# thegenemyers/DEXTRACTOR

Measured on NVIDIA B200. Metric: dexqv+undexqv uncompressed GB/s, higher is better.
Workload: dtype u8

## Files before the change

### dextractor_b200/csrc/dx_api.cpp

```cpp

#include <stdarg.h>
#include <stdio.h>
#include <stdlib.h>
#include <string.h>
#include <vector>
#include <algorithm>
#include <chrono>
#include "dx_internal.h"
#include "dx_chain.h"

struct DxPhases
{ bool on; std::chrono::steady_clock::time_point t0; char buf[512]; size_t len;
  explicit DxPhases(const dx_ctx *ctx) : on(ctx->route[DXR_DEBUG] != 0), len(0) { buf[0] = 0; t0 = std::chrono::steady_clock::now(); }
  void mark(const char *what)
  { if (!on) return;
    auto t1 = std::chrono::steady_clock::now();
    len += (size_t) snprintf(buf+len,sizeof(buf)-len," %s %.3f",what,
                             std::chrono::duration<double,std::milli>(t1-t0).count());
    if (len >= sizeof(buf)) len = sizeof(buf)-1;
    t0 = t1;
  }
  void report(const char *call) { if (on) fprintf(stderr,"[dexb200 debug] %s host phases (ms):%s\n",call,buf); }
};

// ... 114 lines not shown
void dx_prof_begin(dx_ctx *ctx)
{ DxProf *pv = (DxProf *) ctx->prof;
  DxProfRec r; r.name = NULL;
  r.a = pv->get(); r.b = pv->get();
  cudaEventRecord(r.a,ctx->stream);
  pv->push_back(r);
}

void dx_prof_end(dx_ctx *ctx, const char *what)
{ DxProf *pv = (DxProf *) ctx->prof;
  if (pv->empty() || pv->back().name != NULL) return;
  pv->back().name = what;
  cudaEventRecord(pv->back().b,ctx->stream);
}

extern "C" int dx_profile(dx_ctx *ctx, int enable)
{ if (ctx == NULL) return DX_E_ARG;
  if (ctx->prof == NULL) ctx->prof = new DxProf();
  ctx->prof_on = enable ? 1 : 0;
  return DX_OK;
}

extern "C" int dx_profile_report(dx_ctx *ctx, char *buf, size_t cap)
{ if (ctx == NULL || buf == NULL || cap == 0) return DX_E_ARG;
  buf[0] = '\0';
  if (ctx->prof == NULL) return DX_OK;
  DX_CUDA(ctx,cudaStreamSynchronize(ctx->stream));
  DxProf *pv = (DxProf *) ctx->prof;
  struct Acc { const char *name; int calls; double ms; };
  std::vector<Acc> acc;
  for (DxProfRec &r : *pv)
    { float ms = 0;
      if (r.name != NULL && cudaEventElapsedTime(&ms,r.a,r.b) == cudaSuccess)
        { size_t k = 0;
          while (k < acc.size() && strcmp(acc[k].name,r.name) != 0) k++;
          if (k == acc.size()) acc.push_back(Acc{r.name,0,0.0});
          acc[k].calls += 1; acc[k].ms += ms;
        }
      pv->pool.push_back(r.a); pv->pool.push_back(r.b);
    }
  pv->clear();
  size_t at = 0;
  for (const Acc &a : acc)
    { int w = snprintf(buf+at,cap-at,"%s %d %.6f\n",a.name,a.calls,a.ms);
      if (w < 0 || (size_t) w >= cap-at) return dx_fail(ctx,DX_E_CAP,"profile report needs more than %zu bytes",cap);
      at += (size_t) w;
    }
  return DX_OK;
}

extern "C" int dx_open(int device, dx_ctx **out)
{ if (out == NULL) return DX_E_ARG;
  *out = NULL;
  int ndev = 0;
  if (cudaGetDeviceCount(&ndev) != cudaSuccess || ndev <= 0)
    { cudaGetLastError();
      return DX_E_NOGPU;
    }
  if (device < 0 || device >= ndev) return DX_E_ARG;
  if (cudaSetDevice(device) != cudaSuccess) return DX_E_CUDA;
  dx_ctx *ctx = (dx_ctx *) calloc(1,sizeof(dx_ctx));
  if (ctx == NULL) return DX_E_NOMEM;
  ctx->device = device;
  cudaDeviceProp prop;
  if (cudaGetDeviceProperties(&prop,device) != cudaSuccess ||
      cudaStreamCreateWithFlags(&ctx->stream,cudaStreamNonBlocking) != cudaSuccess)
    { free(ctx);
      return DX_E_CUDA;
    }
  ctx->sm_count = prop.multiProcessorCount;
  ctx->route[DXR_DEBUG] = (getenv("DEXB200_DEBUG") != NULL);
  *out = ctx;
  return DX_OK;
}

extern "C" void dx_close(dx_ctx *ctx)
{ if (ctx == NULL) return;
  cudaSetDevice(ctx->device);
  cudaStreamSynchronize(ctx->stream);
  for (int i = 0; i < ctx->nblk; i++) cudaFree(ctx->blk[i].p);
  if (ctx->io_in)    cudaFree(ctx->io_in);
  if (ctx->io_out)   cudaFree(ctx->io_out);
  if (ctx->qv_store) cudaFree(ctx->qv_store);
  if (ctx->last_index) delete (std::vector<dx_index_row> *) ctx->last_index;
  if (ctx->hpin)     cudaFreeHost(ctx->hpin);
  while (ctx->hpin_extra)
    { DxPinExtra *e = (DxPinExtra *) ctx->hpin_extra; ctx->hpin_extra = e->next; cudaFreeHost(e->p); free(e); }
  if (ctx->prof)
    { char tmp[16]; ctx->prof_on = 0; dx_profile_report(ctx,tmp,sizeof(tmp));
      for (cudaEvent_t e : ((DxProf *) ctx->prof)->pool) cudaEventDestroy(e);
      delete (DxProf *) ctx->prof;
    }
  for (int i = 0; i < ctx->npev; i++) cudaEventDestroy(ctx->pev[i]);
  if (ctx->cs_in)  cudaStreamDestroy(ctx->cs_in);
  if (ctx->cs_out) cudaStreamDestroy(ctx->cs_out);
  cudaStreamDestroy(ctx->stream);
  free(ctx);
}

extern "C" const char *dx_strerror(const dx_ctx *ctx) { return ctx ? ctx->err : "no context"; }
extern "C" int64_t     dx_error_line(const dx_ctx *ctx) { return ctx ? ctx->err_line : 0; }
extern "C" size_t      dx_needed_bytes(const dx_ctx *ctx) { return ctx ? ctx->need_bytes : 0; }
extern "C" void       *dx_stream(dx_ctx *ctx) { return ctx ? (void *) ctx->stream : NULL; }

extern "C" int dx_route(dx_ctx *ctx, const char *name, int64_t value)
{ static const char *names[DXR_COUNT] = { "no_fast", "no_spec", "exact_index", "exact_pack", "pack2", "two_pass",
                                          "chain_scan", "decoder", "lane_max_rlen", "lane_min_entries", "debug",
                                          "serial_io", "pipe_chunk", "no_direct", "index_bulk", "hist_mode" };
  if (ctx == NULL || name == NULL) return DX_E_ARG;
  if (strcmp(name,"default") == 0)
    { const int64_t dbg = ctx->route[DXR_DEBUG];
      memset(ctx->route,0,sizeof(ctx->route));
      ctx->route[DXR_DEBUG] = dbg;
      return DX_OK;
    }
  for (int k = 0; k < DXR_COUNT; k++)
    if (strcmp(name,names[k]) == 0) { ctx->route[k] = value; return DX_OK; }
  return dx_fail(ctx,DX_E_ARG,"dx_route: unknown route '%s'",name);
}

extern "C" int dx_keep_index(dx_ctx *ctx, int keep)
{ if (ctx == NULL) return DX_E_ARG;
  ctx->keep_index = keep;
  if (ctx->last_index == NULL) ctx->last_index = new std::vector<dx_index_row>();
  return DX_OK;
}

extern "C" int dx_last_index(dx_ctx *ctx, dx_index_row *rows, int64_t max, int64_t *count)
{ if (ctx == NULL || count == NULL) return DX_E_ARG;
  std::vector<dx_index_row> *v = (std::vector<dx_index_row> *) ctx->last_index;
  *count = v ? (int64_t) v->size() : 0;
  if (v && rows)
    for (int64_t i = 0; i < *count && i < max; i++) rows[i] = (*v)[(size_t) i];
  return DX_OK;
}

extern "C" int dx_sync(dx_ctx *ctx)
{ DX_CUDA(ctx,cudaStreamSynchronize(ctx->stream));
  return DX_OK;
}

extern "C" uint64_t dx_launch_count(dx_ctx *ctx, int reset)
{ uint64_t v = ctx->launches;
  if (reset) ctx->launches = 0;
  return v;
}

extern "C" void *dx_device_alloc(dx_ctx *ctx, size_t bytes)
{ void *p = NULL;
  cudaSetDevice(ctx->device);
  cudaError_t e = cudaMalloc(&p,round_up(bytes + 64,256));
  if (e != cudaSuccess) { dx_cuda_fail(ctx,e,"cudaMalloc"); return NULL; }
  return p;
}
extern "C" void dx_device_free(dx_ctx *ctx, void *p) { (void) ctx; if (p) cudaFree(p); }

extern "C" void *dx_pinned_alloc(dx_ctx *ctx, size_t bytes)
{ void *p = NULL;
  cudaError_t e = cudaHostAlloc(&p,bytes > 0 ? bytes : 1,cudaHostAllocDefault);
  if (e != cudaSuccess) { dx_cuda_fail(ctx,e,"cudaHostAlloc"); return NULL; }
  return p;
}
extern "C" void dx_pinned_free(dx_ctx *ctx, void *p) { (void) ctx; if (p) cudaFreeHost(p); }

extern "C" int dx_h2d(dx_ctx *ctx, void *d, const void *h, size_t n)
{ DX_CUDA(ctx,cudaMemcpyAsync(d,h,n,cudaMemcpyHostToDevice,ctx->stream)); return DX_OK; }
extern "C" int dx_d2d(dx_ctx *ctx, void *d_dst, const void *d_src, size_t n)
{ if (ctx == NULL) return DX_E_ARG;
  cudaSetDevice(ctx->device);
  if (n > 0) DX_CUDA(ctx,cudaMemcpyAsync(d_dst,d_src,n,cudaMemcpyDeviceToDevice,ctx->stream));
  return DX_OK;
}
extern "C" int dx_d2h(dx_ctx *ctx, void *h, const void *d, size_t n)
{ DX_CUDA(ctx,cudaMemcpyAsync(h,d,n,cudaMemcpyDeviceToHost,ctx->stream)); return DX_OK; }


static int check_buf(dx_ctx *ctx, const void *p, const char *what)
{ if (p == NULL) return dx_fail(ctx,DX_E_ARG,"%s is NULL",what);
  if (((uintptr_t) p & 15) != 0)
    return dx_fail(ctx,DX_E_ARG,"%s must be 16-byte aligned device memory",what);
  return DX_OK;
}

static int peek(dx_ctx *ctx, const uint8_t *d, size_t n, size_t at, size_t len, std::vector<uint8_t> &h)
{ if (at > n) at = n;
  if (at + len > n) len = n - at;
  h.resize(len);
  if (len == 0) return DX_OK;
  DX_CUDA(ctx,cudaMemcpyAsync(h.data(),d+at,len,cudaMemcpyDeviceToHost,ctx->stream));
  DX_CUDA(ctx,cudaStreamSynchronize(ctx->stream));
  return DX_OK;
// ... 2059 lines not shown
```

### dextractor_b200/csrc/dx_internal.h

```cpp
#ifndef DX_INTERNAL_H
#define DX_INTERNAL_H

#include <stdint.h>
#include <stddef.h>
#include <cuda_runtime.h>
#include "dexb200.h"


struct QvEntries
{ int64_t  n;
  int64_t *hdr;
  int64_t *line0;
  int32_t *rlen;
  int32_t *well, *beg, *end, *qv;
  int32_t *flag;
  int32_t *order;
};

struct QvSizes
{ uint32_t *bytes;
  int64_t  *off;
};

#define DX_ENC_CODE(e)  ((e) & 0xffffu)
#define DX_ENC_LEN(e)   (((e) >> 16) & 0x1fu)
#define DX_ENC_ESC(e)   (((e) >> 21) & 1u)

struct QvEncTables { uint32_t t[6][256]; };

struct QvDecTables
{ uint8_t look[6][65536];
  uint8_t lens[6][256];
  int32_t type[6];
};

#define DX_DEC2_MAXSUB 64
struct QvDecTables2
{ uint16_t prim[6][2048];
  uint16_t sub[6][DX_DEC2_MAXSUB*32];
  int32_t  type[6];
};

struct QvDecTables4
{ uint32_t multi[6][4096];
  uint16_t single[6][4096];
  float    abits[6];
  QvDecTables2 t2;
  uint32_t longs[6][256];
  int32_t  nlong[6];
};


struct DxBlock { uint8_t *p; size_t cap, top; };

enum { DXR_NO_FAST = 0, DXR_NO_SPEC, DXR_EXACT_INDEX, DXR_EXACT_PACK, DXR_PACK2, DXR_TWO_PASS, DXR_CHAIN_SCAN,
       DXR_DECODER,
       DXR_LANE_MAX_RLEN,
       DXR_LANE_MIN_ENTRIES,
       DXR_DEBUG, DXR_SERIAL_IO,
       DXR_PIPE_CHUNK,
       DXR_NO_DIRECT,
       DXR_INDEX_BULK,
       DXR_HIST_MODE,
       DXR_COUNT };

struct dx_ctx
{ int          device;
  cudaStream_t stream;
  int          sm_count;
  char         err[512];
  int64_t      err_line;
  uint64_t     launches;
  int64_t      route[DXR_COUNT];

  DxBlock      blk[32];
  int          nblk;

  uint8_t     *io_in;   size_t io_in_cap;
  uint8_t     *io_out;  size_t io_out_cap;
  size_t       need_bytes;
  cudaStream_t cs_in, cs_out;
  void       (*overlap_fn)(void *);
  void        *overlap_arg;
  cudaEvent_t  pev[40];
  int          npev;

  int          prof_on;
  void        *prof;

  uint8_t     *hpin;    size_t hpin_cap, hpin_top, hpin_want;
  void        *hpin_extra;

  int          keep_index;
  void        *last_index;

  const uint8_t *qv_text;
  size_t         qv_n;
  QvEntries      qv_ent;
  uint8_t       *qv_store;
  size_t         qv_store_cap;
};

int   dx_fail(dx_ctx *ctx, int code, const char *fmt, ...);
int   dx_cuda_fail(dx_ctx *ctx, cudaError_t e, const char *what);
int   dx_fail_cap(dx_ctx *ctx, size_t need, size_t cap);
void  dx_arena_reset(dx_ctx *ctx);
void *dx_arena_get(dx_ctx *ctx, size_t bytes);
int   dx_arena_reserve(dx_ctx *ctx, size_t bytes);
void *dx_hpin_get(dx_ctx *ctx, size_t bytes);

#define DX_CUDA(ctx, call) do { cudaError_t e__ = (call); \
    if (e__ != cudaSuccess) return dx_cuda_fail(ctx, e__, #call); } while (0)
void dx_prof_begin(dx_ctx *ctx);
void dx_prof_end(dx_ctx *ctx, const char *what);
#define DX_PROF_BEGIN(ctx) do { if ((ctx)->prof_on) dx_prof_begin(ctx); } while (0)
#define DX_LAUNCHED(ctx, what) do { (ctx)->launches++; cudaError_t e__ = cudaGetLastError(); \
    if ((ctx)->prof_on) dx_prof_end(ctx, what); \
    if (e__ != cudaSuccess) return dx_cuda_fail(ctx, e__, what); } while (0)


int dxk_fetch(dx_ctx *ctx, void *h_pinned, const void *d_src, size_t bytes);

enum { DX_PRED_NEWLINE = 0, DX_PRED_FASTA_HDR = 1, DX_PRED_QVCAND = 2, DX_PRED_ARCAND = 3 };
int dxk_index_positions(dx_ctx *ctx, int pred, const uint8_t *d_buf, size_t n, size_t first,
                        int64_t **d_pos, int64_t *count);
int dxk_ticket_order(dx_ctx *ctx, const int32_t *d_rlen, int64_t n, int32_t *d_order);
int dxk_qv_entries(dx_ctx *ctx, const uint8_t *d_text, size_t n, const int64_t *d_nl,
                   int64_t nlines, QvEntries ent, int32_t *h_err, uint64_t *h_totchar,
                   int64_t *h_noncanon, int64_t *h_last_nl);

struct QvProbe
{ int32_t  delchar, subchar;
  int64_t  e_del, e_sub;
  uint64_t sub_prefix[256];
  uint64_t totchar;
};
int dxk_qv_probe(dx_ctx *ctx, const uint8_t *d_text, QvEntries ent, const dx_qv_carry *carry,
                 QvProbe *h_probe);
int dxk_qv_hist(dx_ctx *ctx, const uint8_t *d_text, QvEntries ent, const QvProbe *h_probe,
                uint64_t *h_hist , int32_t *h_newline_inside);

int dxk_qv_encode(dx_ctx *ctx, const uint8_t *d_text, size_t text_n, QvEntries ent,
                  const QvEncTables *h_tab,
                  int delchar, int subchar, int lossy, int32_t lwell_in,
                  uint8_t *d_out, size_t cap, size_t *out_len, int32_t *last_well,
                  int64_t *h_entry_off, int64_t max_entries);

struct QvDecEntry
{ int64_t out_off;
  int64_t text_off;
  int32_t well, beg, end, qv;
};
int dxk_qv_walk(dx_ctx *ctx, const uint8_t *d_in, size_t n, const QvDecTables *d_tab,
                int delchar, int subchar, int flip, const int64_t *d_start, const int32_t *d_rlen,
                int64_t count, int64_t *d_soff, int32_t *d_status );
int dxk_qv_decode(dx_ctx *ctx, const uint8_t *d_in, size_t n, const QvDecTables *d_tab,
                  int delchar, int subchar, int flip, int upper, const QvDecEntry *d_ent,
                  const int64_t *d_soff, int64_t count, const char *d_prefix, int plen,
                  uint8_t *d_out, int32_t *d_status );

int dxk_qv_decode5(dx_ctx *ctx, const uint8_t *d_in, size_t n, const QvDecTables4 *d_tab,
                   int delchar, int subchar, int upper, int write, int64_t count,
                   const int64_t *d_start, const int32_t *d_rlen, const QvDecEntry *d_ent,
                   const char *d_prefix, int plen, uint8_t *d_out, int64_t *d_soff, int32_t *d_status);

int dxk_qv_decode5x(dx_ctx *ctx, const uint8_t *d_in, size_t n, const QvDecTables4 *d_tab,
                    int delchar, int subchar, int upper, int write, int64_t count,
                    const int64_t *d_start, const int32_t *d_rlen, const QvDecEntry *d_ent,
                    const char *d_prefix, int plen, uint8_t *d_out, int64_t *d_soff, int32_t *d_status,
                    const int64_t *d_limit, const int32_t *d_order, const int64_t *d_toff,
                    const int64_t *d_endat = NULL);

int dxk_qv_decode6x(dx_ctx *ctx, const uint8_t *d_in, size_t n, const QvDecTables4 *d_tab,
                    int delchar, int subchar, int upper, int write, int64_t count,
                    const int64_t *d_start, const int32_t *d_rlen, const QvDecEntry *d_ent,
                    const char *d_prefix, int plen, uint8_t *d_out, int64_t *d_soff, int32_t *d_status,
                    const int64_t *d_limit, const int32_t *d_order, const int64_t *d_toff, int64_t n_coop,
                    const int64_t *d_endat = NULL);

int dxk_qv_assemble(dx_ctx *ctx, const uint8_t *d_tmp, size_t tmp_n, const QvDecEntry *d_ent,
                    const int64_t *d_src, int64_t count, const char *d_prefix, int plen, uint8_t *d_out);

struct QvPlanArrays
// ... 92 lines not shown
```

### dextractor_b200/csrc/dx_qv_decode5.cu

```cuda

#include <stdio.h>
#include <stdlib.h>
#include "dx_internal.h"
#include "dx_common.cuh"

namespace {

constexpr int kWarps    = 32;
constexpr int kThreads  = kWarps * 32;
constexpr int kS        = 256;
constexpr int kSW       = kS / 32;
constexpr int kRegion   = kSW + 1;
constexpr int kStage    = 2560;
constexpr int kTail     = 24;
constexpr int kFingerBudget = 24;

struct Dec5Args
{ const uint8_t *in;
  int64_t        n;
  const QvDecTables4 *tab;
  int32_t        delchar, subchar, upper, write;
  int64_t        count;
  const int64_t *start;
  const int32_t *rlen;
  const QvDecEntry *ent;
  const int64_t *toff;
  const char    *prefix; int32_t plen;
  uint8_t       *out;
  int64_t       *soff;
  int32_t       *status;
  const int64_t *limit;
  const int32_t *order;
  const int64_t *endat;
  unsigned long long *ticket;
  unsigned long long *dbg;
};

struct WarpMem
{ uint64_t bits[32*kRegion];
  uint32_t stage[kStage/4 + 4];
};

struct Shared5
{ uint32_t tab[4][4096];
  WarpMem  w[kWarps];
};

extern __shared__ __align__(16) uint8_t dx_dec5_smem[];

__device__ __forceinline__ uint32_t win32(const uint64_t *D, uint32_t pos)
{ const uint64_t v = D[pos >> 5];
  return __funnelshift_l((uint32_t) v,(uint32_t) (v >> 32),pos);
}

__device__ __forceinline__ uint32_t lookup_long(const QvDecTables2 *t, int k, uint32_t w16)
{ uint32_t e = __ldg(&t->prim[k][w16 >> 5]);
  if (e & 0x8000u)
    e = __ldg(&t->sub[k][(e & 0x7fffu)*32u + (w16 & 31u)]);
  return e;
}

__device__ __noinline__ uint32_t long_entry(const QvDecTables2 *t, int k, uint32_t w, uint32_t *bad)
{ const uint32_t f = lookup_long(t,k,w >> 16);
  uint32_t len = (f >> 8) & 31u;
  const uint32_t c = f & 0xffu;
  if (len == 0) { len = 1; *bad = 1; }
  if (t->type[k] == 2 && c == 255u)
    return (len + 8u) | (1u << 5) | 0x80u | (len << 8) | (255u << 16);
  return len | (1u << 5) | (len << 8) | (c << 16);
}

__device__ __noinline__ uint32_t long_single(const QvDecTables2 *t, int k, uint32_t w, uint32_t *bad)
{ uint32_t f = lookup_long(t,k,w >> 16) & 0x1fffu;
  if ((f >> 8) == 0u) { f |= 0x100u; *bad = 1; }
  return f;
}

__device__ __forceinline__ void fill_line(uint8_t *dst, uint32_t c, uint32_t n, uint32_t lane)
{ uint32_t head = (16u - (uint32_t) (reinterpret_cast<uintptr_t>(dst) & 15u)) & 15u;
  if (head > n) head = n;
  if (lane < head) dst[lane] = (uint8_t) c;
  const uint32_t nvec = (n - head) >> 4;
  const uint32_t q = c * 0x01010101u;
  const uint4 v = make_uint4(q,q,q,q);
  uint8_t *body = dst + head;
  for (uint32_t i = lane; i < nvec; i += 32) dx_stg16(body + (size_t) i*16,v);
  const uint32_t done = head + nvec*16u;
  if (lane < n - done) dst[done + lane] = (uint8_t) c;
}

__device__ __forceinline__ void stage_window(const Dec5Args &a, uint64_t *bits, const uint8_t *p,
                                             uint32_t lane, uint32_t nact)
{ if (lane < nact)
    { const uintptr_t A = reinterpret_cast<uintptr_t>(p) + 32u*lane;
      const uint32_t *al = reinterpret_cast<const uint32_t *>(A & ~(uintptr_t) 3);
      const uint32_t sh = (uint32_t) (A & 3) * 8;
      const uint32_t *endw = reinterpret_cast<const uint32_t *>(
                               (reinterpret_cast<uintptr_t>(a.in + a.n) + 3) & ~(uintptr_t) 3);
      uint32_t x[kRegion + 2];
#pragma unroll
      for (int k = 0; k < kRegion + 2; k++) x[k] = (al + k < endw) ? __ldg(al + k) : 0u;
#pragma unroll
      for (int k = 0; k < kRegion; k++)
        { const uint32_t w0 = __funnelshift_r(x[k],x[k+1],sh), w1 = __funnelshift_r(x[k+1],x[k+2],sh);
          bits[kRegion*lane + k] = ((uint64_t) w0 << 32) | w1;
        }
    }
  __syncwarp();
}

#define DX_E_LEN(e)   ((e) & 31u)
#define DX_E_N(e)     (((e) >> 5) & 3u)
#define DX_E_LEN0(e)  (((e) >> 8) & 31u)
#define DX_E_LEN1(e)  (((e) & 0x40u) ? DX_E_LEN0(e) : DX_E_LEN(e))

struct StreamOut { uint32_t bytes, kept, bad; };

template <bool RUN>
__device__ __noinline__ StreamOut decode_stream(const Dec5Args &a, int slot, int64_t so, int32_t rlen,
                                                int symtab, int runtab, int32_t rci, uint8_t *dst,
                                                int64_t budget)
{ Shared5 &sm = *reinterpret_cast<Shared5 *>(dx_dec5_smem);
  const uint32_t lane = threadIdx.x & 31u, warp = threadIdx.x >> 5;
  StreamOut res; res.bytes = 0; res.kept = 0; res.bad = 0;
  if (rlen <= 0)
    { if (dst != NULL && lane == 0) dst[0] = '\n';
      return res;
    }
  const QvDecTables2 *t2 = &a.tab->t2;
  const bool esc = (t2->type[symtab] == 2);
  const uint32_t rc = (uint32_t) rci;
  const uint32_t base = lane * kS, lim = base + kS;
  const float abits = a.tab->abits[symtab] * 1.2f;
  WarpMem &wm = sm.w[warp];
  const uint64_t *D = wm.bits + lane;
  const uint32_t *mt = sm.tab[slot];
  const uint16_t *rt = reinterpret_cast<const uint16_t *>(sm.tab[slot]), *st = rt + 4096;
  uint32_t done = 0;
  uint32_t carry = 0;
  uint32_t wword = 0;
  uint32_t bd = 0, sp = 0, ksum = 0;
  bool redecode = false;
  if (RUN && dst != NULL) fill_line(dst,rc,(uint32_t) rlen,lane);

  while (true)
    { const uint32_t remaining = (uint32_t) rlen - done;
      uint32_t nact = (uint32_t) ((float) remaining * abits * (1.0f/kS)) + 2u;
      if (nact > 32u) nact = 32u;
      const bool active = (lane < nact);
      __syncwarp();
      stage_window(a,wm.bits,a.in + so + (int64_t) wword*4,lane,nact);

      uint32_t mystart = (lane == 0) ? carry : (base << 1);
      uint32_t myexit = 0, n = 0, nk = 0;
      if (active)
        { uint32_t pos = mystart >> 1, cnt = 0, kept = 0;
          if (RUN)
            { uint32_t par = mystart & 1u;
              while (pos < lim)
                { if (par == 0)
                    { uint32_t w = win32(D,pos);
                      uint32_t e = rt[w >> 20];
                      if (e == 0u) e = long_single(t2,runtab,w,&sp);
                      uint32_t r = e & 0xffu;
                      pos += e >> 8;
                      if (r == 255u) { r = win32(D,pos) >> 16; pos += 16; }
                      cnt += r;
                      par = 1;
                      if (pos >= lim) break;
                    }
                  uint32_t w = win32(D,pos);
                  uint32_t e = st[w >> 20];
                  if (e == 0u) e = long_single(t2,symtab,w,&sp);
                  uint32_t c = e & 0xffu;
                  pos += e >> 8;
                  if (esc && c == 255u) { c = win32(D,pos) >> 24; pos += 8; }
                  cnt += 1;
                  kept += (c != rc);
                  par = 0;
                }
              myexit = (pos << 1) | par;
            }
          else
            { const uint32_t limf = lim - kTail;
              while (pos < limf)
                { const uint32_t w = win32(D,pos);
                  uint32_t e = mt[w >> 20];
                  if (e == 0u) e = long_entry(t2,symtab,w,&sp);
                  pos += DX_E_LEN(e);
                  cnt += DX_E_N(e);
                }
              while (pos < lim)
                { const uint32_t w = win32(D,pos);
                  uint32_t e = mt[w >> 20];
                  if (e == 0u) e = long_entry(t2,symtab,w,&sp);
                  pos += DX_E_LEN1(e);
                  cnt += 1;
                }
              myexit = pos << 1;
            }
          n = cnt; nk = kept;
        }

      uint32_t rounds = 0, restarts = 0, slow = 0;
      bool giveup = false;
      while (true)
        { int changed = 0;
          uint32_t want = __shfl_up_sync(DX_FULL,myexit,1);
          if (!active || lane == 0) want = mystart;
          if (want != mystart)
            { uint32_t pa = mystart >> 1, pb = want >> 1, ca = 0, cb = 0, ka = 0, kb = 0;
              restarts++;
              if (RUN)
                { uint32_t qa = mystart & 1u, qb = want & 1u;
                  while (!(pa == pb && qa == qb) && min(pa,pb) < lim)
                    { const bool fa = (pa <= pb);
                      uint32_t pos = fa ? pa : pb, par = fa ? qa : qb, dc, dk = 0;
                      if (par == 0)
                        { uint32_t w = win32(D,pos);
                          uint32_t e = rt[w >> 20];
                          if (e == 0u) e = long_single(t2,runtab,w,&sp);
                          dc = e & 0xffu;
                          pos += e >> 8;
                          if (dc == 255u) { dc = win32(D,pos) >> 16; pos += 16; }
                          par = 1;
                        }
                      else
                        { uint32_t w = win32(D,pos);
                          uint32_t e = st[w >> 20];
                          if (e == 0u) e = long_single(t2,symtab,w,&sp);
                          uint32_t c = e & 0xffu;
                          pos += e >> 8;
                          if (esc && c == 255u) { c = win32(D,pos) >> 24; pos += 8; }
                          dc = 1; dk = (c != rc);
                          par = 0;
                        }
                      if (fa) { pa = pos; qa = par; ca += dc; ka += dk; }
                      else    { pb = pos; qb = par; cb += dc; kb += dk; }
                    }
                  if (pa == pb && qa == qb) { n += cb - ca; nk += kb - ka; }
                  else { n = cb; nk = kb; myexit = (pb << 1) | qb; changed = 1; }
                }
              else if (redecode)
                {
                  uint32_t pos = want >> 1, cnt = 0;
                  const uint32_t limf = lim - kTail;
                  while (pos < limf)
                    { const uint32_t w = win32(D,pos);
                      uint32_t e = mt[w >> 20];
                      if (e == 0u) e = long_entry(t2,symtab,w,&sp);
                      pos += DX_E_LEN(e);
                      cnt += DX_E_N(e);
                    }
                  while (pos < lim)
                    { const uint32_t w = win32(D,pos);
                      uint32_t e = mt[w >> 20];
                      if (e == 0u) e = long_entry(t2,symtab,w,&sp);
                      pos += DX_E_LEN1(e);
                      cnt += 1;
                    }
                  n = cnt;
                  if ((pos << 1) != myexit) { myexit = pos << 1; changed = 1; }
                }
              else
                { uint32_t steps = 0;
                  while (pa != pb && min(pa,pb) < lim)
                    { const bool fa = (pa < pb);
                      const uint32_t pos = fa ? pa : pb;
                      const uint32_t w = win32(D,pos);
                      uint32_t e = mt[w >> 20];
                      if (e == 0u) e = long_entry(t2,symtab,w,&sp);
                      const uint32_t np = pos + DX_E_LEN1(e);
                      if (fa) { pa = np; ca++; } else { pb = np; cb++; }
                      steps++;
                    }
                  if (steps > kFingerBudget) slow = 1;
                  if (pa == pb) n += cb - ca;
                  else { n = cb; myexit = pb << 1; changed = 1; }
                }
              mystart = want;
            }
          rounds++;
          if (!__any_sync(DX_FULL,changed)) break;
          if (a.limit != NULL && rounds >= 12u) { giveup = true; break; }
        }
      if (!RUN && !redecode && __any_sync(DX_FULL,slow != 0)) redecode = true;
      if (giveup)
        { bd = 1;
          res.bytes = wword*4u;
          break;
        }
      if (a.dbg != NULL)
        { if (lane == 0) { atomicAdd(&a.dbg[symtab*4],(unsigned long long) rounds);
                           atomicAdd(&a.dbg[symtab*4+1],1ull); }
          if (restarts) atomicAdd(&a.dbg[symtab*4+3],(unsigned long long) restarts);
        }

      const uint32_t inc = dx_warp_incl_sum(n,lane);
      const uint32_t total = __shfl_sync(DX_FULL,inc,31);
      const uint32_t before = inc - n;
      const bool ends_here = (total >= remaining);
      const bool owner = ends_here && before < remaining && remaining <= before + n;
      uint32_t need = 0;
      if (before < remaining) need = min(n,remaining - before);

      const bool wr = (dst != NULL);
      const uint32_t outn = min(total,remaining);
      const bool staged = wr && !RUN && outn <= (uint32_t) kStage;
      uint32_t last = 0, kfin = 0;
      if (need > 0 && (wr || owner))
        { uint8_t *p;
          if (staged) p = reinterpret_cast<uint8_t *>(wm.stage) + before;
          else        p = dst + done + before;
          uint32_t pos = mystart >> 1, cnt = 0;
          if (RUN)
            { uint32_t par = mystart & 1u;
              while (cnt < need)
                { if (par == 0)
                    { uint32_t w = win32(D,pos);
                      uint32_t e = rt[w >> 20];
                      if (e == 0u) e = long_single(t2,runtab,w,&bd);
                      uint32_t r = e & 0xffu;
                      last = pos;
                      pos += e >> 8;
                      if (r == 255u) { r = win32(D,pos) >> 16; last = pos; pos += 16; }
                      if (r > need - cnt) { r = need - cnt; bd = 1; }
                      cnt += r; p += r;
                      par = 1;
                      if (cnt >= need) break;
                    }
                  uint32_t w = win32(D,pos);
                  uint32_t e = st[w >> 20];
                  if (e == 0u) e = long_single(t2,symtab,w,&bd);
                  uint32_t c = e & 0xffu;
                  last = pos;
                  pos += e >> 8;
                  if (esc && c == 255u) { c = win32(D,pos) >> 24; last = pos; pos += 8; }
                  if (wr) *p = (uint8_t) c;
                  p++; cnt++;
                  kfin += (c != rc);
                  par = 0;
                }
            }
          else
            {
              while (cnt + 2u < need)
                { const uint32_t w = win32(D,pos);
                  uint32_t e = mt[w >> 20];
                  if (e == 0u) e = long_entry(t2,symtab,w,&bd);
                  uint32_t c0 = (e >> 16) & 0xffu;
                  if (e & 0x80u) c0 = (w << DX_E_LEN0(e)) >> 24;
                  if (wr)
                    { p[0] = (uint8_t) c0;
                      if (e & 0x40u) p[1] = (uint8_t) (e >> 24);
                    }
                  pos += DX_E_LEN(e);
                  p   += DX_E_N(e);
                  cnt += DX_E_N(e);
                }
              while (cnt < need)
                { const uint32_t w = win32(D,pos);
                  uint32_t e = mt[w >> 20];
                  if (e == 0u) e = long_entry(t2,symtab,w,&bd);
                  uint32_t c0 = (e >> 16) & 0xffu;
                  const uint32_t l0 = DX_E_LEN0(e);
                  last = pos;
                  if (e & 0x80u) { c0 = (w << l0) >> 24; last = pos + l0; }
                  if (wr) p[0] = (uint8_t) c0;
                  pos += (e & 0x80u) ? l0 + 8u : l0;
                  p++; cnt++;
                }
            }
        }
      if (RUN && symtab == 0)
        { uint32_t contrib = 0;
          if (owner) contrib = kfin;
          else if (need == n && n > 0) contrib = nk;
          ksum += dx_warp_sum(contrib);
        }
      if (staged)
        { __syncwarp();
          dx_warp_copy_out(dst + done,wm.stage,outn,lane);
        }
      if (ends_here)
        { const uint32_t who = __ffs(__ballot_sync(DX_FULL,owner)) - 1;
          const uint32_t endw = (wword*32u + last + 47u) >> 5;
          res.bytes = __shfl_sync(DX_FULL,endw,who & 31u) * 4u;
          break;
        }
      done  += total;
      carry  = __shfl_sync(DX_FULL,myexit,nact-1) - ((nact*kS) << 1);
      wword += nact*kSW;
      if (so + (int64_t) wword*4 > budget + 8)
        { bd = 1;
          res.bytes = wword*4u;
          break;
        }
    }
  __syncwarp();
  if (a.dbg != NULL && lane == 0) atomicAdd(&a.dbg[symtab*4+2],1ull);
  if (dst != NULL && lane == 0) dst[rlen] = '\n';
  res.kept = ksum;
  res.bad  = __any_sync(DX_FULL,bd != 0);
  return res;
}

__device__ __noinline__ void write_tags(const Dec5Args &a, const uint8_t *del, const uint8_t *packed,
                                        int32_t rlen, uint8_t *dst)
{ Shared5 &sm = *reinterpret_cast<Shared5 *>(dx_dec5_smem);
  const uint32_t lane = threadIdx.x & 31u, warp = threadIdx.x >> 5;
  uint32_t *stw = sm.w[warp].stage;
  uint8_t  *stb = reinterpret_cast<uint8_t *>(stw);
  const uint32_t caseoff = a.upper ? 32u : 0u;
  const uint32_t nn = ('n' - caseoff) * 0x01010101u;
  uint32_t rank = 0;
  for (int32_t p0 = 0; p0 < rlen; p0 += 512)
    { const int32_t p = p0 + (int32_t) lane*16;
      const int cnt = max(0,min(16,rlen - p));
      uint32_t m = 0;
      if (cnt > 0)
        { if (a.delchar < 0) m = (1u << cnt) - 1u;
          else
            {
              const uintptr_t A = reinterpret_cast<uintptr_t>(del + p);
              const uint32_t *al = reinterpret_cast<const uint32_t *>(A & ~(uintptr_t) 3);
              const uint32_t *endw = reinterpret_cast<const uint32_t *>(
                                       (reinterpret_cast<uintptr_t>(del + rlen) + 3) & ~(uintptr_t) 3);
              const uint32_t sh = (uint32_t) (A & 3) * 8;
              uint32_t x[5];
#pragma unroll
              for (int k = 0; k < 5; k++) x[k] = (al + k < endw) ? __ldcg(al + k) : 0u;
              const uint4 d = make_uint4(__funnelshift_r(x[0],x[1],sh),__funnelshift_r(x[1],x[2],sh),
                                         __funnelshift_r(x[2],x[3],sh),__funnelshift_r(x[3],x[4],sh));
              m = ~dx_eq_mask16(d,(uint32_t) a.delchar) & ((1u << cnt) - 1u);
            }
        }
      const uint32_t c = __popc(m);
      const uint32_t inc = dx_warp_incl_sum(c,lane);
      uint32_t r = rank + inc - c;
      rank += __shfl_sync(DX_FULL,inc,31);
      stw[4*lane] = nn; stw[4*lane+1] = nn; stw[4*lane+2] = nn; stw[4*lane+3] = nn;
      while (m)
        { const int k = __ffs(m) - 1; m &= m - 1;
          const uint32_t byte = __ldg(packed + (r >> 2));
          const uint32_t ch = (0x74676361u >> (8*((byte >> (6 - 2*(r & 3))) & 3u))) & 0xffu;
          stb[16*lane + k] = (uint8_t) (ch - caseoff);
          r++;
        }
      __syncwarp();
      dx_warp_copy_out(dst + p0,stw,(uint32_t) min(512,rlen - p0),lane);
      __syncwarp();
    }
  if (lane == 0) dst[rlen] = '\n';
}

__device__ int fmt_int5(uint8_t *p, int32_t v)
{ char tmp[12];
  int  k = 0, len = 0;
  uint32_t u = (v < 0) ? (uint32_t) (-(int64_t) v) : (uint32_t) v;
  if (v < 0) p[len++] = '-';
  do { tmp[k++] = (char) ('0' + u % 10); u /= 10; } while (u);
  while (k) p[len++] = (uint8_t) tmp[--k];
  return len;
}

__global__ void __launch_bounds__(kThreads,1)
k_qv_decode5(Dec5Args a)
{ Shared5 &sm = *reinterpret_cast<Shared5 *>(dx_dec5_smem);
  const uint32_t lane = threadIdx.x & 31u;

  { const QvDecTables4 *T = a.tab;
    for (int s = 0; s < 4; s++)
      { const int symtab = (s == 0) ? 0 : (s == 1) ? 2 : (s == 2) ? 3 : 4;
        const int runtab = (s == 0) ? 1 : 5;
        const bool run = (s == 0 && a.delchar >= 0) || (s == 3 && a.subchar >= 0);
        if (run)
          { const uint32_t *gr = reinterpret_cast<const uint32_t *>(T->single[runtab]);
            const uint32_t *gs = reinterpret_cast<const uint32_t *>(T->single[symtab]);
            for (int j = threadIdx.x; j < 2048; j += kThreads)
              { sm.tab[s][j] = __ldg(gr + j); sm.tab[s][2048 + j] = __ldg(gs + j); }
          }
        else
          for (int j = threadIdx.x; j < 4096; j += kThreads) sm.tab[s][j] = __ldg(T->multi[symtab] + j);
// ... 88 lines not shown
};

__global__ void __launch_bounds__(256)
k_qv_assemble(AsmArgs a)
{ const uint32_t lane = threadIdx.x & 31u;
  const int64_t nwarp = ((int64_t) gridDim.x * blockDim.x) >> 5;
  for (int64_t e = ((int64_t) blockIdx.x * blockDim.x + threadIdx.x) >> 5; e < a.count; e += nwarp)
    { const int64_t so = a.src[e];
      if (so < 0) continue;
      const QvDecEntry en = a.ent[e];
      if (lane == 0)
        { uint8_t *h = a.out + en.out_off;
          int hl = 0;
          for (int k = 0; k < a.plen; k++) h[hl++] = (uint8_t) a.prefix[k];
          h[hl++] = '/'; hl += fmt_int5(h+hl,en.well);
          h[hl++] = '/'; hl += fmt_int5(h+hl,en.beg);
          h[hl++] = '_'; hl += fmt_int5(h+hl,en.end);
          const char *rq = " RQ=0.";
          for (int k = 0; k < 6; k++) h[hl++] = (uint8_t) rq[k];
          hl += fmt_int5(h+hl,en.qv);
          h[hl++] = '\n';
        }
      const int64_t n = 5*((int64_t) en.end - en.beg + 1);
      uint8_t *dst = a.out + en.text_off;
      const uint8_t *src = a.tmp + so;
      int64_t head = (16 - (int64_t) (reinterpret_cast<uintptr_t>(dst) & 15)) & 15;
      if (head > n) head = n;
      if ((int64_t) lane < head) dst[lane] = src[lane];
      const int64_t nvec = (n - head) >> 4;
      for (int64_t i = lane; i < nvec; i += 32)
        dx_stg16(dst + head + i*16,dx_ld16_any(src + head + i*16,a.tmp_end16));
      const int64_t done = head + nvec*16;
      if ((int64_t) lane < n - done) dst[done + lane] = src[done + lane];
    }
}

}

int dxk_qv_assemble(dx_ctx *ctx, const uint8_t *d_tmp, size_t tmp_n, const QvDecEntry *d_ent,
                    const int64_t *d_src, int64_t count, const char *d_prefix, int plen, uint8_t *d_out)
{ if (count == 0) return DX_OK;
  AsmArgs a;
  a.tmp = d_tmp; a.tmp_end16 = d_tmp + ((tmp_n + 15) & ~(size_t) 15);
  a.ent = d_ent; a.src = d_src; a.count = count; a.prefix = d_prefix; a.plen = plen; a.out = d_out;
  int64_t grid = (count + 7) / 8;
  if (grid > (int64_t) ctx->sm_count * 8) grid = (int64_t) ctx->sm_count * 8;
  DX_PROF_BEGIN(ctx); k_qv_assemble<<<(unsigned) grid,256,0,ctx->stream>>>(a);
  DX_LAUNCHED(ctx,"k_qv_assemble");
  return DX_OK;
}

int dxk_qv_decode5x(dx_ctx *ctx, const uint8_t *d_in, size_t n, const QvDecTables4 *d_tab,
                    int delchar, int subchar, int upper, int write, int64_t count,
                    const int64_t *d_start, const int32_t *d_rlen, const QvDecEntry *d_ent,
                    const char *d_prefix, int plen, uint8_t *d_out, int64_t *d_soff, int32_t *d_status,
                    const int64_t *d_limit, const int32_t *d_order, const int64_t *d_toff,
                    const int64_t *d_endat);

int dxk_qv_decode5(dx_ctx *ctx, const uint8_t *d_in, size_t n, const QvDecTables4 *d_tab,
                   int delchar, int subchar, int upper, int write, int64_t count,
                   const int64_t *d_start, const int32_t *d_rlen, const QvDecEntry *d_ent,
                   const char *d_prefix, int plen, uint8_t *d_out, int64_t *d_soff, int32_t *d_status)
{ return dxk_qv_decode5x(ctx,d_in,n,d_tab,delchar,subchar,upper,write,count,d_start,d_rlen,d_ent,d_prefix,plen,
                         d_out,d_soff,d_status,NULL,NULL,NULL,NULL);
}

int dxk_qv_decode5x(dx_ctx *ctx, const uint8_t *d_in, size_t n, const QvDecTables4 *d_tab,
                    int delchar, int subchar, int upper, int write, int64_t count,
                    const int64_t *d_start, const int32_t *d_rlen, const QvDecEntry *d_ent,
                    const char *d_prefix, int plen, uint8_t *d_out, int64_t *d_soff, int32_t *d_status,
                    const int64_t *d_limit, const int32_t *d_order, const int64_t *d_toff,
                    const int64_t *d_endat)
{ if (count == 0) return DX_OK;
  unsigned long long *d_ticket = (unsigned long long *) dx_arena_get(ctx,8);
  if (d_ticket == NULL) return DX_E_NOMEM;
  DX_CUDA(ctx,cudaMemsetAsync(d_ticket,0,8,ctx->stream));
  Dec5Args a;
  a.in = d_in; a.n = (int64_t) n; a.tab = d_tab;
  a.delchar = delchar; a.subchar = subchar; a.upper = upper; a.write = write;
  a.count = count; a.start = d_start; a.rlen = d_rlen; a.ent = d_ent;
  a.prefix = d_prefix; a.plen = plen; a.out = d_out; a.soff = d_soff; a.status = d_status;
  a.ticket = d_ticket;
  a.limit = d_limit; a.order = d_order; a.toff = d_toff; a.endat = d_endat;
  a.dbg = NULL;
  const size_t smem = sizeof(Shared5);
  DX_CUDA(ctx,cudaFuncSetAttribute(k_qv_decode5,cudaFuncAttributeMaxDynamicSharedMemorySize,(int) smem));
  int64_t grid = (count + kWarps - 1) / kWarps;
  if (grid > ctx->sm_count) grid = ctx->sm_count;
  DX_PROF_BEGIN(ctx); k_qv_decode5<<<(unsigned) grid,kThreads,smem,ctx->stream>>>(a);
  DX_LAUNCHED(ctx,write == 1 ? "k_qv_decode5" : write >= 2 ? "k_qv_decode5_spec" : "k_qv_walk5");
  return DX_OK;
}
```

Before: 431.1.

## Record decoded symbols during counting pass and copy them instead of re-decoding

During the counting pass of the QV decoder, each lane now stores its decoded symbols in a per-lane global scratch buffer, packed four bytes per word with stride-32 interleaving. The write phase then re-decodes only up to a junction point and copies the rest from the buffer with funnel shifts, so most symbols are no longer Huffman-decoded twice. In exchange, every counting step now does extra global stores through L2, and a persistent scratch buffer is allocated per SM. A debug-counter route is also added to report how many lanes take the copy path versus the re-decode path.

```diff
diff --git a/dextractor_b200/csrc/dx_api.cpp b/dextractor_b200/csrc/dx_api.cpp
--- a/dextractor_b200/csrc/dx_api.cpp
+++ b/dextractor_b200/csrc/dx_api.cpp
@@ -220,6 +220,7 @@
   if (ctx->io_in)    cudaFree(ctx->io_in);
   if (ctx->io_out)   cudaFree(ctx->io_out);
   if (ctx->qv_store) cudaFree(ctx->qv_store);
+  if (ctx->dec5_slots) cudaFree(ctx->dec5_slots);
   if (ctx->last_index) delete (std::vector<dx_index_row> *) ctx->last_index;
   if (ctx->hpin)     cudaFreeHost(ctx->hpin);
   while (ctx->hpin_extra)
@@ -244,7 +245,8 @@
 extern "C" int dx_route(dx_ctx *ctx, const char *name, int64_t value)
 { static const char *names[DXR_COUNT] = { "no_fast", "no_spec", "exact_index", "exact_pack", "pack2", "two_pass",
                                           "chain_scan", "decoder", "lane_max_rlen", "lane_min_entries", "debug",
-                                          "serial_io", "pipe_chunk", "no_direct", "index_bulk", "hist_mode" };
+                                          "serial_io", "pipe_chunk", "no_direct", "index_bulk", "hist_mode",
+                                          "dec5_counters" };
   if (ctx == NULL || name == NULL) return DX_E_ARG;
   if (strcmp(name,"default") == 0)
     { const int64_t dbg = ctx->route[DXR_DEBUG];
diff --git a/dextractor_b200/csrc/dx_internal.h b/dextractor_b200/csrc/dx_internal.h
--- a/dextractor_b200/csrc/dx_internal.h
+++ b/dextractor_b200/csrc/dx_internal.h
@@ -62,6 +62,7 @@
        DXR_NO_DIRECT,
        DXR_INDEX_BULK,
        DXR_HIST_MODE,
+       DXR_DEC5_COUNTERS,
        DXR_COUNT };
 
 struct dx_ctx
@@ -99,6 +100,9 @@
   QvEntries      qv_ent;
   uint8_t       *qv_store;
   size_t         qv_store_cap;
+
+  uint32_t      *dec5_slots;
+  size_t         dec5_slots_cap;
 };
 
 int   dx_fail(dx_ctx *ctx, int code, const char *fmt, ...);
diff --git a/dextractor_b200/csrc/dx_qv_decode5.cu b/dextractor_b200/csrc/dx_qv_decode5.cu
--- a/dextractor_b200/csrc/dx_qv_decode5.cu
+++ b/dextractor_b200/csrc/dx_qv_decode5.cu
@@ -14,6 +14,9 @@
 constexpr int kStage    = 2560;
 constexpr int kTail     = 24;
 constexpr int kFingerBudget = 24;
+constexpr int kSlotWords = 66;
+constexpr int kDbg      = 6;
+constexpr int kCopyBatch = 8;
 
 struct Dec5Args
 { const uint8_t *in;
@@ -34,6 +37,7 @@
   const int64_t *endat;
   unsigned long long *ticket;
   unsigned long long *dbg;
+  uint32_t      *slots;
 };
 
 struct WarpMem
@@ -116,6 +120,69 @@
 
 struct StreamOut { uint32_t bytes, kept, bad; };
 
+
+__device__ __forceinline__ uint32_t slot_put(uint32_t *sl, uint32_t acc, uint32_t cnt, uint32_t e, uint32_t w,
+                                             uint32_t nsym)
+{ uint32_t v = (e & 0x80u) ? (w << DX_E_LEN0(e)) >> 24 : e >> 16;
+  if (nsym == 1u) v &= 0xffu;
+  const uint32_t b = (cnt & 3u) * 8u;
+  const uint64_t t = ((uint64_t) v << b) | acc;
+  if (b + 8u*nsym >= 32u)
+    { __stcg(sl + 32u*(cnt >> 2),(uint32_t) t);
+      return (uint32_t) (t >> 32);
+    }
+  return (uint32_t) t;
+}
+
+template <bool REC>
+__device__ __forceinline__ uint32_t count_plain(const uint64_t *D, uint32_t pos, uint32_t lim, const uint32_t *mt,
+                                                const QvDecTables2 *t2, int symtab, uint32_t *bad, uint32_t *sl,
+                                                uint32_t &cnt)
+{ uint32_t c = 0, acc = 0;
+  const uint32_t limf = lim - kTail;
+  while (pos < limf)
+    { const uint32_t w = win32(D,pos);
+      uint32_t e = mt[w >> 20];
+      if (e == 0u) e = long_entry(t2,symtab,w,bad);
+      if (REC) acc = slot_put(sl,acc,c,e,w,DX_E_N(e));
+      pos += DX_E_LEN(e);
+      c   += DX_E_N(e);
+    }
+  while (pos < lim)
+    { const uint32_t w = win32(D,pos);
+      uint32_t e = mt[w >> 20];
+      if (e == 0u) e = long_entry(t2,symtab,w,bad);
+      if (REC) acc = slot_put(sl,acc,c,e,w,1u);
+      pos += DX_E_LEN1(e);
+      c   += 1;
+    }
+  if (REC && (c & 3u)) __stcg(sl + 32u*(c >> 2),acc);
+  cnt = c;
+  return pos;
+}
+
+__device__ __forceinline__ void slot_copy(const uint32_t *sl, uint32_t s, uint8_t *stb, uint32_t d, uint32_t m)
+{ uint32_t h = (4u - (d & 3u)) & 3u;
+  if (h > m) h = m;
+  const uint32_t nw = (m - h) >> 2, q = s + h, sh = (q & 3u) * 8u;
+  const uint32_t qt = q + 4u*nw, t = m - h - 4u*nw;
+  const uint32_t hv = __funnelshift_r(__ldcg(sl + 32u*(s >> 2)),__ldcg(sl + 32u*((s >> 2) + 1)),(s & 3u)*8u);
+  const uint32_t tv = __funnelshift_r(__ldcg(sl + 32u*(qt >> 2)),__ldcg(sl + 32u*((qt >> 2) + 1)),(qt & 3u)*8u);
+  const uint32_t *src = sl + 32u*(q >> 2);
+  uint32_t *dw = reinterpret_cast<uint32_t *>(stb + d + h);
+  uint32_t lo = __ldcg(src);
+  for (uint32_t j0 = 0; j0 < nw; j0 += kCopyBatch)
+    { uint32_t x[kCopyBatch];
+#pragma unroll
+      for (int u = 0; u < kCopyBatch; u++) x[u] = (j0 + u < nw) ? __ldcg(src + 32u*(j0 + u + 1)) : 0u;
+#pragma unroll
+      for (int u = 0; u < kCopyBatch; u++)
+        if (j0 + u < nw) { dw[j0 + u] = __funnelshift_r(lo,x[u],sh); lo = x[u]; }
+    }
+  for (uint32_t k = 0; k < h; k++) stb[d + k] = (uint8_t) (hv >> 8u*k);
+  for (uint32_t k = 0; k < t; k++) stb[d + h + 4u*nw + k] = (uint8_t) (tv >> 8u*k);
+}
+
 template <bool RUN>
 __device__ __noinline__ StreamOut decode_stream(const Dec5Args &a, int slot, int64_t so, int32_t rlen,
                                                 int symtab, int runtab, int32_t rci, uint8_t *dst,
@@ -141,6 +208,8 @@
   uint32_t wword = 0;
   uint32_t bd = 0, sp = 0, ksum = 0;
   bool redecode = false;
+  const bool rec = !RUN && dst != NULL;
+  uint32_t *sl = rec ? a.slots + (size_t) (blockIdx.x*kWarps + warp)*(kSlotWords*32) + lane : NULL;
   if (RUN && dst != NULL) fill_line(dst,rc,(uint32_t) rlen,lane);
 
   while (true)
@@ -153,6 +222,7 @@
 
       uint32_t mystart = (lane == 0) ? carry : (base << 1);
       uint32_t myexit = 0, n = 0, nk = 0;
+      uint32_t jm = mystart >> 1, js = 0, jp = 0;
       if (active)
         { uint32_t pos = mystart >> 1, cnt = 0, kept = 0;
           if (RUN)
@@ -182,22 +252,12 @@
               myexit = (pos << 1) | par;
             }
           else
-            { const uint32_t limf = lim - kTail;
-              while (pos < limf)
-                { const uint32_t w = win32(D,pos);
-                  uint32_t e = mt[w >> 20];
-                  if (e == 0u) e = long_entry(t2,symtab,w,&sp);
-                  pos += DX_E_LEN(e);
-                  cnt += DX_E_N(e);
-                }
-              while (pos < lim)
-                { const uint32_t w = win32(D,pos);
-                  uint32_t e = mt[w >> 20];
-                  if (e == 0u) e = long_entry(t2,symtab,w,&sp);
-                  pos += DX_E_LEN1(e);
-                  cnt += 1;
-                }
+            { uint32_t b = 0;
+              if (rec) pos = count_plain<true >(D,pos,lim,mt,t2,symtab,&b,sl,cnt);
+              else     pos = count_plain<false>(D,pos,lim,mt,t2,symtab,&b,sl,cnt);
               myexit = pos << 1;
+              sp |= b;
+              if (b) jm = ~0u;
             }
           n = cnt; nk = kept;
         }
@@ -243,22 +303,11 @@
                 }
               else if (redecode)
                 {
-                  uint32_t pos = want >> 1, cnt = 0;
-                  const uint32_t limf = lim - kTail;
-                  while (pos < limf)
-                    { const uint32_t w = win32(D,pos);
-                      uint32_t e = mt[w >> 20];
-                      if (e == 0u) e = long_entry(t2,symtab,w,&sp);
-                      pos += DX_E_LEN(e);
-                      cnt += DX_E_N(e);
-                    }
-                  while (pos < lim)
-                    { const uint32_t w = win32(D,pos);
-                      uint32_t e = mt[w >> 20];
-                      if (e == 0u) e = long_entry(t2,symtab,w,&sp);
-                      pos += DX_E_LEN1(e);
-                      cnt += 1;
-                    }
+                  uint32_t pos, cnt, b = 0;
+                  if (rec) pos = count_plain<true >(D,want >> 1,lim,mt,t2,symtab,&b,sl,cnt);
+                  else     pos = count_plain<false>(D,want >> 1,lim,mt,t2,symtab,&b,sl,cnt);
+                  sp |= b;
+                  jm = b ? ~0u : want >> 1; js = 0; jp = 0;
                   n = cnt;
                   if ((pos << 1) != myexit) { myexit = pos << 1; changed = 1; }
                 }
@@ -275,8 +324,14 @@
                       steps++;
                     }
                   if (steps > kFingerBudget) slow = 1;
-                  if (pa == pb) n += cb - ca;
-                  else { n = cb; myexit = pb << 1; changed = 1; }
+                  if (pa == pb)
+                    { n += cb - ca;
+                      if (jm != ~0u)
+                        { if (ca >= jp) { js += ca - jp; jm = pa; jp = cb; }
+                          else jp += cb - ca;
+                        }
+                    }
+                  else { n = cb; myexit = pb << 1; changed = 1; jm = ~0u; }
                 }
               mystart = want;
             }
@@ -291,9 +346,9 @@
           break;
         }
       if (a.dbg != NULL)
-        { if (lane == 0) { atomicAdd(&a.dbg[symtab*4],(unsigned long long) rounds);
-                           atomicAdd(&a.dbg[symtab*4+1],1ull); }
-          if (restarts) atomicAdd(&a.dbg[symtab*4+3],(unsigned long long) restarts);
+        { if (lane == 0) { atomicAdd(&a.dbg[symtab*kDbg],(unsigned long long) rounds);
+                           atomicAdd(&a.dbg[symtab*kDbg+1],1ull); }
+          if (restarts) atomicAdd(&a.dbg[symtab*kDbg+3],(unsigned long long) restarts);
         }
 
       const uint32_t inc = dx_warp_incl_sum(n,lane);
@@ -308,7 +363,30 @@
       const uint32_t outn = min(total,remaining);
       const bool staged = wr && !RUN && outn <= (uint32_t) kStage;
       uint32_t last = 0, kfin = 0;
-      if (need > 0 && (wr || owner))
+      const bool copy = staged && !owner && jm != ~0u;
+      if (a.dbg != NULL && staged)
+        { const uint32_t cp = __popc(__ballot_sync(DX_FULL,need > 0 && copy));
+          const uint32_t rd = __popc(__ballot_sync(DX_FULL,need > 0 && !copy));
+          if (lane == 0) { atomicAdd(&a.dbg[symtab*kDbg+4],(unsigned long long) cp);
+                           atomicAdd(&a.dbg[symtab*kDbg+5],(unsigned long long) rd); }
+        }
+      if (need > 0 && copy)
+        { uint8_t *stb = reinterpret_cast<uint8_t *>(wm.stage);
+          uint32_t pos = mystart >> 1, c = 0;
+          while (c < need && pos < jm)
+            { const uint32_t w = win32(D,pos);
+              uint32_t e = mt[w >> 20];
+              if (e == 0u) e = long_entry(t2,symtab,w,&bd);
+              uint32_t c0 = (e >> 16) & 0xffu;
+              const uint32_t l0 = DX_E_LEN0(e);
+              if (e & 0x80u) c0 = (w << l0) >> 24;
+              stb[before + c] = (uint8_t) c0;
+              pos += (e & 0x80u) ? l0 + 8u : l0;
+              c++;
+            }
+          slot_copy(sl,js,stb,before + c,need - c);
+        }
+      else if (need > 0 && (wr || owner))
         { uint8_t *p;
           if (staged) p = reinterpret_cast<uint8_t *>(wm.stage) + before;
           else        p = dst + done + before;
@@ -398,7 +476,7 @@
         }
     }
   __syncwarp();
-  if (a.dbg != NULL && lane == 0) atomicAdd(&a.dbg[symtab*4+2],1ull);
+  if (a.dbg != NULL && lane == 0) atomicAdd(&a.dbg[symtab*kDbg+2],1ull);
   if (dst != NULL && lane == 0) dst[rlen] = '\n';
   res.kept = ksum;
   res.bad  = __any_sync(DX_FULL,bd != 0);
@@ -653,11 +731,22 @@
   a.prefix = d_prefix; a.plen = plen; a.out = d_out; a.soff = d_soff; a.status = d_status;
   a.ticket = d_ticket;
   a.limit = d_limit; a.order = d_order; a.toff = d_toff; a.endat = d_endat;
-  a.dbg = NULL;
+  a.dbg = (unsigned long long *) (uintptr_t) ctx->route[DXR_DEC5_COUNTERS];
   const size_t smem = sizeof(Shared5);
   DX_CUDA(ctx,cudaFuncSetAttribute(k_qv_decode5,cudaFuncAttributeMaxDynamicSharedMemorySize,(int) smem));
   int64_t grid = (count + kWarps - 1) / kWarps;
   if (grid > ctx->sm_count) grid = ctx->sm_count;
+  a.slots = NULL;
+  if (write)
+    { const size_t need = (size_t) ctx->sm_count*kWarps*32*kSlotWords*4;
+      if (ctx->dec5_slots_cap < need)
+        { if (ctx->dec5_slots) cudaFree(ctx->dec5_slots);
+          ctx->dec5_slots = NULL; ctx->dec5_slots_cap = 0;
+          DX_CUDA(ctx,cudaMalloc((void **) &ctx->dec5_slots,need));
+          ctx->dec5_slots_cap = need;
+        }
+      a.slots = ctx->dec5_slots;
+    }
   DX_PROF_BEGIN(ctx); k_qv_decode5<<<(unsigned) grid,kThreads,smem,ctx->stream>>>(a);
   DX_LAUNCHED(ctx,write == 1 ? "k_qv_decode5" : write >= 2 ? "k_qv_decode5_spec" : "k_qv_walk5");
   return DX_OK;
```

Result: slower. 407.4 (median of 6 runs) (-5.5%).
